# xiph/rav1e

Measured on AMD Instinct MI355X. Metric: RDO-candidate Mpixels/s (dist+fwd_tx+mc) at 4K speed-6, higher is better.
Workload: dtype u8

## Files before the change

rav1e_amd/csrc/cand_common.hpp:

```cpp
#pragma once
#include <type_traits>

#include "common.hpp"
#include "dist_common.hpp"
#include "mc_common.hpp"

namespace r1cand {

#include "mc_taps_packed.inc"

template <int CTRL>
__device__ __forceinline__ int32_t dpp(int32_t x) {
  return __builtin_amdgcn_update_dpp(0, x, CTRL, 0xf, 0xf, true);
}
template <int CTRL>
__device__ __forceinline__ int32_t bfly_lanes(int32_t x, int32_t sm) {
  return __mul24(x, sm | 1) + dpp<CTRL>(x);
}
struct LaneSigns { int32_t s1, s2; };
template <int TS>
__device__ __forceinline__ LaneSigns lane_signs(int lane) {
  LaneSigns s;
  if constexpr (TS == 8) {
    s.s1 = -(int32_t)((lane ^ (lane >> 2)) & 1);
    s.s2 = -(int32_t)(((lane >> 1) ^ (lane >> 2)) & 1);
  } else {
    s.s1 = -(int32_t)(lane & 1);
    s.s2 = 0;
  }
  return s;
}
template <int TS>
__device__ __forceinline__ uint32_t habs_lanes(int32_t x, LaneSigns sg) {
  x = bfly_lanes<0xB1>(x, sg.s1);
  if constexpr (TS == 8) x = bfly_lanes<0x4E>(x, sg.s2);
  const int32_t ax = iabs32(x);
  const int32_t ap = TS == 8 ? dpp<0x141>(ax) : dpp<0x4E>(ax);
  return (uint32_t)(ax > ap ? ax : ap);
}

__device__ __forceinline__ uint32_t sad_u32(uint32_t a, uint32_t b, uint32_t acc) {
  uint32_t r;
  asm("v_sad_u32 %0, %1, %2, %3" : "=v"(r) : "v"(a), "v"(b), "v"(acc));
  return r;
}

typedef short v2s_t __attribute__((ext_vector_type(2)));
typedef unsigned short v2us_t __attribute__((ext_vector_type(2)));
__device__ __forceinline__ uint32_t pk_add(uint32_t a, uint32_t b) {
  return __builtin_bit_cast(uint32_t, (v2s_t)(__builtin_bit_cast(v2s_t, a) + __builtin_bit_cast(v2s_t, b)));
}
__device__ __forceinline__ uint32_t pk_sub(uint32_t a, uint32_t b) {
  return __builtin_bit_cast(uint32_t, (v2s_t)(__builtin_bit_cast(v2s_t, a) - __builtin_bit_cast(v2s_t, b)));
}
__device__ __forceinline__ uint32_t pk_mad(uint32_t x, uint32_t s, uint32_t p) {
  uint32_t r;
  asm("v_pk_mad_i16 %0, %1, %2, %3" : "=v"(r) : "v"(x), "v"(s), "v"(p));
  return r;
}
__device__ __forceinline__ uint32_t pk_max(uint32_t a, uint32_t b) {
  uint32_t r;
  asm("v_pk_max_i16 %0, %1, %2" : "=v"(r) : "v"(a), "v"(b));
  return r;
}
__device__ __forceinline__ uint32_t pk_min(uint32_t a, uint32_t b) {
  uint32_t r;
  asm("v_pk_min_i16 %0, %1, %2" : "=v"(r) : "v"(a), "v"(b));
  return r;
}
__device__ __forceinline__ uint32_t pk_pair(int32_t lo, int32_t hi) {
  return __builtin_amdgcn_perm((uint32_t)hi, (uint32_t)lo, 0x05040100u);
}
__device__ __forceinline__ void pk_bfly8_s2(const uint32_t (&a)[8], uint32_t (&d)[8]) {
  uint32_t b[8];
#pragma unroll
  for (int k = 0; k < 4; k++) {
    b[2 * k] = pk_add(a[2 * k], a[2 * k + 1]);
    b[2 * k + 1] = pk_sub(a[2 * k], a[2 * k + 1]);
  }
  d[0] = pk_add(b[0], b[2]); d[2] = pk_sub(b[0], b[2]);
  d[1] = pk_add(b[1], b[3]); d[3] = pk_sub(b[1], b[3]);
  d[4] = pk_add(b[4], b[6]); d[6] = pk_sub(b[4], b[6]);
  d[5] = pk_add(b[5], b[7]); d[7] = pk_sub(b[5], b[7]);
}
__device__ __forceinline__ uint32_t habs_lanes_pk(uint32_t x, uint32_t m1, uint32_t m2, uint32_t acc) {
  x = pk_mad(x, m1, (uint32_t)dpp<0xB1>((int32_t)x));
  x = pk_mad(x, m2, (uint32_t)dpp<0x4E>((int32_t)x));
  const uint32_t ax = pk_max(x, pk_sub(0u, x));
  const uint32_t mx = pk_max(ax, (uint32_t)dpp<0x141>((int32_t)ax));
  return __builtin_amdgcn_udot2(__builtin_bit_cast(v2us_t, mx), __builtin_bit_cast(v2us_t, 0x00010001u),
                                acc, false);
}

__device__ __forceinline__ uint32_t ashr_pair(int32_t lo, int32_t hi, int sh) {
  return __builtin_amdgcn_perm((uint32_t)(hi >> sh), (uint32_t)(lo >> sh), 0x05040100u);
}

__device__ __forceinline__ int32_t dot2_seed0(uint32_t a, uint32_t b) {
  int32_t r;
  asm("v_dot2_i32_i16 %0, %1, %2, 0" : "=v"(r) : "v"(a), "v"(b));
  return r;
}
__device__ __forceinline__ int32_t dot2_seed64(uint32_t a, uint32_t b) {
  int32_t r;
  asm("v_dot2_i32_i16 %0, %1, %2, 64" : "=v"(r) : "v"(a), "v"(b));
  return r;
}
__device__ __forceinline__ int32_t dot2_seed(uint32_t a, uint32_t b, int32_t c_uniform) {
  int32_t r;
  asm("v_dot2_i32_i16 %0, %1, %2, %3" : "=v"(r) : "v"(a), "v"(b), "s"(c_uniform));
  return r;
}
__device__ __forceinline__ int32_t dot4_seed(uint32_t a, uint32_t b, int32_t c_uniform) {
  int32_t r;
  asm("v_dot4_i32_i8 %0, %1, %2, %3" : "=v"(r) : "v"(a), "v"(b), "s"(c_uniform));
  return r;
}

template <int BPP> struct Taps;
template <> struct Taps<1> { uint32_t fx0, fx1, ty[4]; };
template <> struct Taps<2> { uint32_t tx[4], ty[4]; };
template <int BPP, int W, int H>
__device__ __forceinline__ Taps<BPP> load_taps(int cf, int rf, int mx, int my) {
  const int fxi = r1mc::filter_index(mx, W), fyi = r1mc::filter_index(my, H);
  Taps<BPP> t;
  if constexpr (BPP == 1) {
    t.fx0 = kTapI8[fxi][cf][0];
    t.fx1 = kTapI8[fxi][cf][1];
  }
#pragma unroll
  for (int j = 0; j < 4; j++) {
    if constexpr (BPP == 2) t.tx[j] = kTapI16[fxi][cf][j];
    t.ty[j] = kTapI16[fyi][rf][j];
  }
  return t;
}
__device__ __forceinline__ bool taps_six(const Taps<1> &t) {
  return __all(((t.ty[0] & 0xffffu) | (t.ty[3] >> 16)) == 0);
}
__device__ __forceinline__ bool taps_six(const Taps<2> &t) {
  return __all(((t.ty[0] & 0xffffu) | (t.ty[3] >> 16) | (t.tx[0] & 0xffffu) | (t.tx[3] >> 16)) == 0);
}

#define R1_ODD_ROW_TAPS(ty, tz)                                                                   \
  do {                                                                                            \
    tz[0] = ty[0] << 16;                                                                          \
    _Pragma("unroll") for (int j = 1; j < 4; j++) tz[j] = __builtin_amdgcn_alignbit(ty[j], ty[j - 1], 16); \
    tz[4] = ty[3] >> 16;                                                                          \
  } while (0)

typedef int v4i_t __attribute__((ext_vector_type(4)));
template <int W, int H, int WS, bool PREP, bool PACK4 = false, int MXNC = 0, bool MX4 = false>
__device__ __forceinline__ void mc8_column_t(const uint8_t *win, int c, const Taps<1> &tp, int32_t *pred, bool six,
                                             int lane = 0, const uint8_t *zero = nullptr) {
  const uint32_t fx0 = tp.fx0, fx1 = tp.fx1;
  uint32_t ty[4], tz[5];
#pragma unroll
  for (int j = 0; j < 4; j++) ty[j] = tp.ty[j];
// ... 141 lines not shown
    auto hpair = [&](int r) -> uint32_t {
      if (r + 1 < H + 7) return ashr_pair(hacc(r), hacc(r + 1), hsh);
      return (uint32_t)(hacc(r) >> hsh);
    };
    uint32_t pk[5];
    pk[0] = SIX ? (uint32_t)(hacc(1) >> hsh) << 16 : hpair(0);
#pragma unroll
    for (int j = 1; j < 4; j++) pk[j] = hpair(2 * j);
#pragma unroll
    for (int j = 0; j < H / 2; j++) {
      if (!SIX || j + 1 < H / 2) pk[4] = hpair(2 * j + 8);
      int32_t a0 = PREP ? dot2_seed64(pk[0], ty[0]) : dot2_seed0(pk[0], ty[0]);
#pragma unroll
      for (int k = 1; k < 4; k++)
        a0 = __builtin_amdgcn_sdot2(__builtin_bit_cast(v2s_t, pk[k]), __builtin_bit_cast(v2s_t, ty[k]), a0, false);
      int32_t a1;
      if constexpr (SIX) {
        a1 = PREP ? dot2_seed64(pk[1], tz[1]) : dot2_seed0(pk[1], tz[1]);
#pragma unroll
        for (int k = 2; k < 4; k++)
          a1 = __builtin_amdgcn_sdot2(__builtin_bit_cast(v2s_t, pk[k]), __builtin_bit_cast(v2s_t, tz[k]), a1, false);
      } else {
        a1 = PREP ? dot2_seed64(pk[0], tz[0]) : dot2_seed0(pk[0], tz[0]);
#pragma unroll
        for (int k = 1; k < 5; k++)
          a1 = __builtin_amdgcn_sdot2(__builtin_bit_cast(v2s_t, pk[k]), __builtin_bit_cast(v2s_t, tz[k]), a1, false);
      }
      if constexpr (PREP) {
        pred[2 * j] = (a0 >> 7) - 8192;
        pred[2 * j + 1] = (a1 >> 7) - 8192;
      } else {
        a0 >>= vsh;
        a1 >>= vsh;
        pred[2 * j] = a0 < 0 ? 0 : (a0 > maxv ? maxv : a0);
        pred[2 * j + 1] = a1 < 0 ? 0 : (a1 > maxv ? maxv : a1);
      }
#pragma unroll
      for (int k = 0; k < 4; k++) pk[k] = pk[k + 1];
    }
  };
  if (six) body(std::true_type{});
  else body(std::false_type{});
}

template <int BPP, int W, int H, int WS, bool PREP, bool PACK4 = false, int MXNC = 0, bool MX4 = false>
__device__ __forceinline__ void mc_column_fast(const uint8_t *win, int c, const Taps<BPP> &tp, int bit_depth,
                                               int32_t *pred, bool six, int lane = 0, const uint8_t *zero = nullptr) {
  static_assert(!PACK4 || BPP == 1, "8 * mid of 16-bit pixels does not fit i16");
  static_assert((MXNC == 0 && !MX4) || BPP == 1, "there is no i16 matrix type");
  if constexpr (BPP == 1) mc8_column_t<W, H, WS, PREP, PACK4, MXNC, MX4>(win, c, tp, pred, six, lane, zero);
  else mc16_column_t<W, H, WS, PREP>(win, c, tp, bit_depth, pred, six);
}

__device__ __forceinline__ void satd_rows16_s2(const int32_t *v, uint32_t (&d)[8]) {
  uint32_t a[8];
#pragma unroll
  for (int k = 0; k < 8; k++) a[k] = pk_pair(v[k], v[8 + k]);
  pk_bfly8_s2(a, d);
}
template <int W, int H>
__device__ __forceinline__ void satd_tile_store(const int32_t *v, uint32_t *tcol) {
#pragma unroll
  for (int g = 0; g < H / 16; g++) {
    uint32_t d[8];
    satd_rows16_s2(v + g * 16, d);
#pragma unroll
    for (int k = 0; k < 4; k++) {
      tcol[(g * 8 + 2 * k) * W] = pk_add(d[k], d[k + 4]);
      tcol[(g * 8 + 2 * k + 1) * W] = pk_sub(d[k], d[k + 4]);
    }
  }
}
template <int NI, int P>
__device__ __forceinline__ uint32_t satd_tile_rows(const uint32_t *tile, int c) {
  uint32_t acc = 0;
#pragma unroll
  for (int m = 0; m < NI; m++) {
    const uint4 *p = (const uint4 *)(tile + (c + m * P) * 8);
    const uint4 lo = p[0], hi = p[1];
    const uint32_t x[8] = {lo.x, lo.y, lo.z, lo.w, hi.x, hi.y, hi.z, hi.w};
    uint32_t z[8];
    pk_bfly8_s2(x, z);
#pragma unroll
    for (int k = 0; k < 4; k++) {
      const uint32_t mx = pk_max(pk_max(z[k], z[k + 4]), pk_sub(0u, pk_min(z[k], z[k + 4])));
      acc = __builtin_amdgcn_udot2(__builtin_bit_cast(v2us_t, mx), __builtin_bit_cast(v2us_t, 0x00020002u), acc, false);
    }
  }
  return acc;
}

template <int TS, int H, int BD>
__device__ __forceinline__ uint32_t satd_column(const int32_t *v, int lane) {
  const LaneSigns sg = lane_signs<TS>(lane);
  uint32_t acc = 0;
  if constexpr (TS == 8 && BD <= 10) {
    const uint32_t m1 = (uint32_t)sg.s1 | 0x00010001u, m2 = (uint32_t)sg.s2 | 0x00010001u;
    if constexpr (H == 8) {
      uint32_t a[4];
#pragma unroll
      for (int k = 0; k < 4; k++) a[k] = pk_pair(v[k] + v[k + 4], v[k] - v[k + 4]);
      const uint32_t a0 = pk_add(a[0], a[1]), a1 = pk_sub(a[0], a[1]);
      const uint32_t a2 = pk_add(a[2], a[3]), a3 = pk_sub(a[2], a[3]);
      acc = habs_lanes_pk(pk_add(a0, a2), m1, m2, acc);
      acc = habs_lanes_pk(pk_add(a1, a3), m1, m2, acc);
      acc = habs_lanes_pk(pk_sub(a0, a2), m1, m2, acc);
      acc = habs_lanes_pk(pk_sub(a1, a3), m1, m2, acc);
    } else {
#pragma unroll
      for (int g = 0; g < H / 16; g++) {
        uint32_t d[8];
        satd_rows16_s2(v + g * 16, d);
#pragma unroll
        for (int k = 0; k < 4; k++) {
          acc = habs_lanes_pk(pk_add(d[k], d[k + 4]), m1, m2, acc);
          acc = habs_lanes_pk(pk_sub(d[k], d[k + 4]), m1, m2, acc);
        }
      }
    }
    return acc;
  }
#pragma unroll
  for (int g = 0; g < H / TS; g++) {
    int32_t a[TS];
#pragma unroll
    for (int k = 0; k < TS; k++) a[k] = v[g * TS + k];
    if constexpr (TS == 4) {
      const int32_t a0 = a[0] + a[1], a1 = a[0] - a[1];
      const int32_t a2 = a[2] + a[3], a3 = a[2] - a[3];
      a[0] = a0 + a2; a[1] = a1 + a3; a[2] = a0 - a2; a[3] = a1 - a3;
    } else {
      int32_t b[8], d[8];
#pragma unroll
      for (int k = 0; k < 4; k++) {
        b[2 * k] = a[2 * k] + a[2 * k + 1];
        b[2 * k + 1] = a[2 * k] - a[2 * k + 1];
      }
      d[0] = b[0] + b[2]; d[2] = b[0] - b[2];
      d[1] = b[1] + b[3]; d[3] = b[1] - b[3];
      d[4] = b[4] + b[6]; d[6] = b[4] - b[6];
      d[5] = b[5] + b[7]; d[7] = b[5] - b[7];
#pragma unroll
      for (int k = 0; k < 4; k++) {
        a[k] = d[k] + d[k + 4];
        a[k + 4] = d[k] - d[k + 4];
      }
    }
#pragma unroll
    for (int k = 0; k < TS; k++) acc += habs_lanes<TS>(a[k], sg);
  }
  return acc;
}

}
```

rav1e_amd/csrc/rdo_cand_kernel.hpp:

```cpp
#pragma once
#include <cstdlib>
#include <type_traits>

#include "cand_common.hpp"
#include "dist_common.hpp"
#include "intra_pred_common.hpp"
#include "itx_common.hpp"
#include "mc_common.hpp"
#include "quant_common.hpp"
#include "rdo_cand_args.hpp"
#include "tx_common.hpp"

#ifdef R1_PHASE_PROF
static __device__ unsigned long long g_phase[4096][8];
#define R1_PROF(i)                                                          \
  do {                                                                      \
    const unsigned long long t_ = __builtin_readcyclecounter();             \
    if (QM == 0 && threadIdx.x == 0 && (blockIdx.x & 63) == 0 && (blockIdx.x >> 6) < 4096) \
      g_phase[blockIdx.x >> 6][i] = t_ - tprev_;                            \
    tprev_ = t_;                                                            \
  } while (0)
#define R1_PROF_INIT unsigned long long tprev_ = __builtin_readcyclecounter()
#else
#define R1_PROF(i) do {} while (0)
#define R1_PROF_INIT do {} while (0)
#endif

namespace {
using r1tx::T;
using r1cand::sad_u32;

template <int BD, int WL, int HL, typename CT, int QM, bool MT = false, int PS = 0>
__global__ __launch_bounds__(64, rdo_waves_hint(BD, WL, HL, QM, MT)) void k_rdo_cand(
    R1Plane org, R1Plane ref, const R1RdoCand *__restrict__ cands, int n,
    uint32_t *__restrict__ sad_out, uint32_t *__restrict__ satd_out,
    CT *__restrict__ coeffs, void *__restrict__ pred_out, RdoQuantArgs qa,
    typename std::conditional<PS == 1, RdoIntraArgs, RdoNoIntraArgs>::type ia) {
  using PL = RdoCandPlan<BD, WL, HL, QM, MT, PS>;
  constexpr int BPP = PL::BPP, W = PL::W, H = PL::H, P = PL::P, NC = PL::NC, TS = PL::TS, WS = PL::WS, FL = PL::FL, HU = PL::HU;
  constexpr bool INTRA = PL::INTRA, SPLIT_T = PL::SPLIT_T, SRC_LDS = PL::SRC_LDS, SRC_LATE = PL::SRC_LATE,
                 SRC_KEEP = PL::SRC_KEEP, SATD_T = PL::SATD_T, COLSHARE = PL::COLSHARE;
  typedef typename PL::TB TB;
  constexpr int LSTRIDE = PL::LSTRIDE, ISTRIDE = PL::ISTRIDE, QT_STRIDE = PL::QT_STRIDE, SRC_ROW = PL::SRC_ROW,
                SRC_CSTRIDE = PL::SRC_CSTRIDE, SATD_STRIDE = PL::SATD_STRIDE, LDS_WORK = PL::LDS_WORK,
                SRC_OFF = PL::SRC_OFF, TKEEP_OFF = PL::TKEEP_OFF, LDS_BYTES = PL::LDS_BYTES;
  static_assert(!INTRA || LDS_BYTES <= RdoCandPlan<BD, WL, HL, QM, MT, 0>::LDS_BYTES,
                "an intra instantiation's LDS must not exceed its inter twin's");
  constexpr int SH0 = r1tx::fwd_shift_ct(WL, HL, BD, 0), SH1 = r1tx::fwd_shift_ct(WL, HL, BD, 1),
                SH2 = r1tx::fwd_shift_ct(WL, HL, BD, 2);
  constexpr bool COL_FOLD = PL::COL_FOLD;
  static_assert(!COL_FOLD || SH0 > 0, "the column family starts from a pending shift[0]");
  constexpr int SH1C = COL_FOLD ? 0 : SH1;
  constexpr bool HALVE2 = PL::HALVE2, MC_PACK4 = PL::MC_PACK4;
  constexpr bool MUL_HW = PL::MUL_HW;
  constexpr int CB = rdo_mul_col_bound(BD, SH0, COL_FOLD), RB = rdo_mul_row_bound(BD, WL, HL);
  constexpr int MX_NC = PL::MX_NC;
  static_assert(MX_NC == 0 || (BPP == 1 && QM == 0 && !INTRA && P == W && NC * W == 64),
                "a coefficient kernel of 8-bit pixels, lane = (candidate, column) with no idle lane");
  constexpr bool MC_MATRIX4 = PL::MC_MATRIX4;
  static_assert(!MC_MATRIX4 || (BPP == 1 && QM == 0 && !INTRA && P == W && NC * W == 64),
                "a coefficient kernel of 8-bit pixels, lane = (candidate, column) with no idle lane");
  __shared__ __attribute__((aligned(16))) uint8_t smem[LDS_BYTES];
  T *buf = (T *)smem;
  TB *tbuf = (TB *)smem;
  TB *tkeep = COLSHARE ? (TB *)(smem + TKEEP_OFF) : tbuf;

  R1_PROF_INIT;
  const unsigned wg = xcd_contiguous_wg();
  if ((long long)wg * NC >= (long long)n) return;
  const int lane = threadIdx.x;
  const int cl = lane / P, c = lane % P;
  const int cand_i = (int)wg * NC + cl;
  const long long cand = cand_i;
  constexpr bool UNMASK = !(BD == 8 && WL == 6 && HL == 6);
  const bool live_st = cand_i < n;
  static_assert(!MC_MATRIX4 || UNMASK, "the 4x4x4 MFMAs take operands from all 64 lanes: dead slots repeat a candidate");
  const bool live = UNMASK || live_st;
  const int cl_ld = live_st ? cl : n - 1 - (int)wg * NC;
  const long long cand_ld = live_st ? cand : (long long)n - 1;
  R1RdoCand cd = {};
  R1IntraCand ic = {};
  int eset = 0;
  if constexpr (INTRA) {
    if (live) {
      ic = ia.cands[cand_ld];
      eset = (int)cand_ld / ia.edge_group;
      cd.ox = ia.pos_xy[2 * eset];
      cd.oy = ia.pos_xy[2 * eset + 1];
    }
  } else {
    if (live) cd = (cands + (size_t)wg * NC)[cl_ld];
  }
#ifdef R1_PHASE_PROF
  asm volatile("s_waitcnt vmcnt(0)" ::: "memory");
  R1_PROF(5);
#endif
  constexpr bool QUANT = QM != 0;
  constexpr int PPK = QM == 2 ? (H * BPP + 3) / 4 : 1;
  uint32_t ppk[PPK];
#pragma unroll
  for (int k = 0; k < PPK; k++) ppk[k] = 0;

  T v[H];
#pragma unroll
  for (int r = 0; r < H; r++) v[r] = 0;
  const bool col_live = live && c < W;
  const uint8_t *src_l = smem + SRC_OFF + cl * SRC_CSTRIDE + c * BPP;
  constexpr int CHS = SRC_ROW >= 16 ? 16 : SRC_ROW;
  constexpr int CPR = SRC_ROW / CHS;
  constexpr int RPP = P / CPR;
  constexpr int SPASS = SRC_LDS ? (H + RPP - 1) / RPP : 1;
  const int srow = c / CPR, sch = c - srow * CPR;
  U32x4 q[SPASS];
  if constexpr (SRC_LDS) {
    const uint8_t *po = (const uint8_t *)org.data +
                        (((uint32_t)(org.yorigin + cd.oy) * (uint32_t)org.stride + (uint32_t)(org.xorigin + cd.ox)) * BPP +
                         (uint32_t)(sch * CHS));
    const uint32_t so = (uint32_t)org.stride * BPP;
#pragma unroll
    for (int u = 0; u < SPASS; u++) {
      const int rr = srow + u * RPP;
      q[u] = U32x4{0, 0, 0, 0};
      if (live && rr < H) {
        if constexpr (CHS == 16) q[u] = ld_u32x4(po + rr * so);
        else if constexpr (CHS == 8) { const U32x2 t = ld_u32x2(po + rr * so); q[u].a = t.a; q[u].b = t.b; }
        else q[u].a = ld_u32(po + rr * so);
      }
    }
  } else if (col_live) {
    const uint8_t *po = px_addr<BPP>(org, cd.ox + c, cd.oy);
    const size_t so = (size_t)org.stride * BPP;
#pragma unroll
    for (int r = 0; r < H; r++) v[r] = ld_px<BPP>(po + r * so);
  }
  uint8_t *win = smem + cl * (H + 7) * WS;
  const bool from_ref = !INTRA && live && !qa.pred_in;
  r1mc::WindowStage<BPP, BPP == 1 ? 0x80808080u : 0u, W, H, P> wst;
  if (from_ref) wst.load(ref, cd.rx, cd.ry, c);
  r1cand::Taps<BPP> tp = {};
  if (from_ref) tp = r1cand::load_taps<BPP, W, H>(cd.col_frac, cd.row_frac, cd.mode_x, cd.mode_y);
  const bool six = r1cand::taps_six(tp);
  if constexpr (PL::MX_ZERO_BYTES != 0) {
#pragma unroll
    for (int k = 0; k < (PL::MX_ZERO_BYTES / 16 + 63) / 64; k++)
      if (lane + 64 * k < PL::MX_ZERO_BYTES / 16)
        *(uint4 *)(smem + PL::MX_ZERO_OFF + 16 * (lane + 64 * k)) = make_uint4(0u, 0u, 0u, 0u);
  }
  auto stage_source = [&]() {
    if (live) {
      uint8_t *sd = smem + SRC_OFF + cl * SRC_CSTRIDE + sch * CHS;
#pragma unroll
      for (int u = 0; u < SPASS; u++) {
        const int rr = srow + u * RPP;
        if (rr < H) {
          if constexpr (CHS == 16) *(uint4 *)(sd + rr * SRC_ROW) = make_uint4(q[u].a, q[u].b, q[u].c, q[u].d);
          else if constexpr (CHS == 8) *(uint2 *)(sd + rr * SRC_ROW) = make_uint2(q[u].a, q[u].b);
          else *(uint32_t *)(sd + rr * SRC_ROW) = q[u].a;
        }
      }
    }
  };
  if constexpr (SRC_LDS && !SRC_LATE && !INTRA) stage_source();
  if (from_ref) wst.store(win, WS);
  uint16_t *eraw = (uint16_t *)smem + cl * (5 * FL);
  int left_len = 0, above_len = 0;
  if constexpr (INTRA) {
    if (live) {
      left_len = ia.lens[2 * eset];
      above_len = ia.lens[2 * eset + 1];
      const uint8_t *e = (const uint8_t *)ia.edges + ((size_t)eset * ia.edge_stride + (2 * r1ip::MAXTX - (W + H))) * BPP;
      for (int k = c; k < FL; k += P) eraw[k] = (uint16_t)ld_px<BPP>(e + k * BPP);
    }
  }
#ifdef R1_PHASE_PROF
  asm volatile("s_waitcnt vmcnt(0)" ::: "memory");
  R1_PROF(6);
#endif
  __syncthreads();
  R1_PROF(0);

  uint32_t sad_acc = 0;
  if constexpr (INTRA) {
    const bool directional = live && r1ip::is_directional(ic.mode, ic.angle);
    const bool enable = directional && ic.ief != 0;
    const uint16_t *tl = eraw + (W + H);
    uint16_t *work = eraw + FL;
    int up_a = 0, up_l = 0;
    r1ip::edge_filter_upsample<const R1IntraCand &>(tl, 0, work, W, H, P, c, ic, enable, left_len, above_len,
                                                     (1 << BD) - 1, up_a, up_l);
    int32_t pred[H];
    if (col_live) {
      if (ic.mode == r1ip::UV_CFL_PRED && !ia.ac) ic.angle = 0;
      const int16_t *acb = ic.mode == r1ip::UV_CFL_PRED && ia.ac ? ia.ac + (size_t)cand_ld * (W * H) : nullptr;
      r1ip::predict_column<const R1IntraCand &>(W, H, c, ic, directional, enable, up_a, up_l, tl, 0, work, left_len, BD,
                                                 acb, [&](int i, int32_t pv) { pred[i] = pv; });
      if (pred_out && live_st) {
        if constexpr (BPP == 1) {
          uint8_t *pp = (uint8_t *)pred_out + (size_t)cand * W * H + c;
#pragma unroll
          for (int r = 0; r < H; r++) pp[(size_t)r * W] = (uint8_t)pred[r];
        } else {
          uint16_t *pp = (uint16_t *)pred_out + (size_t)cand * W * H + c;
#pragma unroll
          for (int r = 0; r < H; r++) pp[(size_t)r * W] = (uint16_t)pred[r];
        }
      }
      if constexpr (QM == 2) {
#pragma unroll
        for (int r = 0; r < H; r++) {
          if constexpr (BPP == 1) ppk[r >> 2] |= (uint32_t)pred[r] << (8 * (r & 3));
          else ppk[r >> 1] |= (uint32_t)pred[r] << (16 * (r & 1));
        }
      }
    }
    if constexpr (SRC_LDS) {
      __syncthreads();
      stage_source();
      __syncthreads();
    }
    if (col_live) {
      if constexpr (SRC_LDS) {
#pragma unroll
        for (int r = 0; r < H; r++) {
          const uint32_t sp = BPP == 1 ? (uint32_t)src_l[r * SRC_ROW] : (uint32_t) * (const uint16_t *)(src_l + r * SRC_ROW);
          sad_acc = sad_u32(sp, (uint32_t)pred[r], sad_acc);
          v[r] = (T)sp - pred[r];
        }
      } else {
#pragma unroll
        for (int r = 0; r < H; r++) v[r] -= pred[r];
      }
    }
  } else
  if constexpr (BPP == 1) {
    if (col_live) {
      int32_t pred[H];
      if (qa.pred_in) {
        const uint8_t *pi = (const uint8_t *)qa.pred_in + (size_t)cand_ld * W * H + c;
#pragma unroll
        for (int r = 0; r < H; r++) pred[r] = pi[(size_t)r * W];
      } else {
        if constexpr (MX_NC != 0)
          r1cand::mc_column_fast<BPP, W, H, WS, false, MC_PACK4, MX_NC>(smem, c, tp, BD, pred, six, lane,
                                                                         smem + PL::MX_ZERO_OFF);
        else if constexpr (MC_MATRIX4)
          r1cand::mc_column_fast<BPP, W, H, WS, false, MC_PACK4, 0, true>(win, c, tp, BD, pred, six);
        else
        r1cand::mc_column_fast<BPP, W, H, WS, false, MC_PACK4>(win, c, tp, BD, pred, six);
      }
      if (pred_out && live_st) {
        uint8_t *pp = (uint8_t *)pred_out + (size_t)cand * W * H + c;
#pragma unroll
        for (int r = 0; r < H; r++) pp[(size_t)r * W] = (uint8_t)pred[r];
      }
      if constexpr (QM == 2) {
#pragma unroll
        for (int r = 0; r < H; r++) ppk[r >> 2] |= (uint32_t)pred[r] << (8 * (r & 3));
      }
      if constexpr (SRC_LDS) {
#pragma unroll
        for (int r = 0; r < H; r++) {
          const uint32_t sp = src_l[r * SRC_ROW];
          sad_acc = sad_u32(sp, (uint32_t)pred[r], sad_acc);
          v[r] = (T)sp - pred[r];
        }
      } else {
#pragma unroll
        for (int r = 0; r < H; r++) v[r] -= pred[r];
      }
    }
  } else {
    int32_t pred[H];
    if (col_live) {
      if (qa.pred_in) {
        const uint16_t *pi = (const uint16_t *)qa.pred_in + (size_t)cand_ld * W * H + c;
#pragma unroll
        for (int r = 0; r < H; r++) pred[r] = pi[(size_t)r * W];
      } else {
        r1cand::mc_column_fast<BPP, W, H, WS, false>(win, c, tp, BD, pred, six);
      }
      if (pred_out && live_st) {
        uint16_t *pp = (uint16_t *)pred_out + (size_t)cand * W * H + c;
#pragma unroll
        for (int r = 0; r < H; r++) pp[(size_t)r * W] = (uint16_t)pred[r];
      }
      if constexpr (QM == 2) {
#pragma unroll
        for (int r = 0; r < H; r++) ppk[r >> 1] |= (uint32_t)pred[r] << (16 * (r & 1));
      }
    }
    if constexpr (SRC_LATE) {
      __syncthreads();
      stage_source();
      __syncthreads();
    }
    if (col_live) {
      if constexpr (SRC_LDS) {
#pragma unroll
        for (int r = 0; r < H; r++) {
          const uint32_t sp = *(const uint16_t *)(src_l + r * SRC_ROW);
          sad_acc = sad_u32(sp, (uint32_t)pred[r], sad_acc);
          v[r] = (T)sp - pred[r];
        }
      } else {
#pragma unroll
        for (int r = 0; r < H; r++) v[r] -= pred[r];
      }
    }
  }
  R1_PROF(1);
  if (sad_out) {
    uint32_t sad = sad_acc;
    if constexpr (!SRC_LDS) {
#pragma unroll
      for (int r = 0; r < H; r++) sad += (uint32_t)iabs32(v[r]);
    }
    const uint32_t s = group_sum<P>(sad);
    if (live_st && c == 0) (sad_out + (size_t)wg * NC)[cl] = s;
  }
  if (satd_out) {
    uint32_t part;
    if constexpr (SATD_T) {
      uint32_t *tile = (uint32_t *)smem + cl * SATD_STRIDE;
      __syncthreads();
      if (c < W) r1cand::satd_tile_store<W, H>(v, tile + c);
      __syncthreads();
      part = r1cand::satd_tile_rows<(W < H ? W : H) / 16, P>(tile, c);
    } else {
      part = r1cand::satd_column<TS, H, BD>(v, lane);
    }
    const uint32_t s = group_sum<P>(part);
    constexpr int LN = TS == 4 ? 2 : 3;
    if (live_st && c == 0) (satd_out + (size_t)wg * NC)[cl] = (s + ((1u << LN) >> 1)) >> LN;
  }
  R1_PROF(2);
  if (!QUANT && !coeffs) return;

  constexpr bool MT_RECOMP = MT && SRC_KEEP;
  T vkeep[MT && !MT_RECOMP ? H : 1];
  if constexpr (MT && !MT_RECOMP) {
#pragma unroll
    for (int r = 0; r < H; r++) vkeep[r] = v[r];
  }
  constexpr bool TAIL_DEFER = MT && QM == 2 && W == 8 && H == 8;
  const bool tail_defer = TAIL_DEFER && qa.dist_kind == R1_DIST_CDEF && qa.nt <= 8;
  r1dist::CdefMoments tail_keep;
  uint32_t rem = MT ? qa.tx_mask : 1u;
  bool fresh = true;
  do {
  int t0 = 0;
  uint32_t gmask = 1u;
  if constexpr (MT) {
    t0 = (int)__builtin_ctz(rem);
    gmask = 1u << t0;
    if constexpr (COLSHARE) {
      auto colkey = [](int t) { return r1tx::vtx_1d(t) | ((int)r1tx::ud_flip(t) << 4) | ((int)r1tx::lr_flip(t) << 5); };
      const int k0 = colkey(t0);
      for (uint32_t m = rem & (rem - 1); m != 0; m &= m - 1) {
        const int t = (int)__builtin_ctz(m);
        if (colkey(t) == k0) gmask |= 1u << t;
      }
    }
    rem &= ~gmask;
    if (!fresh) {
      if constexpr (MT_RECOMP) {
        if (col_live) {
#pragma unroll
          for (int r = 0; r < H; r++) {
            const T sp = BPP == 1 ? (T)src_l[r * SRC_ROW] : (T) * (const uint16_t *)(src_l + r * SRC_ROW);
            const T pr = BPP == 1 ? (T)((ppk[r >> 2] >> (8 * (r & 3))) & 0xFF)
                                  : (T)((ppk[r >> 1] >> (16 * (r & 1))) & 0xFFFF);
            v[r] = sp - pr;
          }
        }
      } else {
#pragma unroll
        for (int r = 0; r < H; r++) v[r] = vkeep[r];
      }
    }
    fresh = false;
  }
  __syncthreads();
  const int tx_col = MT ? t0 : (QM != 0 && qa.tx_mask != 0 ? (int)__builtin_ctz(qa.tx_mask) : (int)cd.tx_type);
  constexpr bool TX_VOTE = rdo_tx_vote(WL, HL, QM, MT, PS);
  static_assert(!TX_VOTE || UNMASK, "the vote reads every lane's descriptor");
  int tx_s = 0;
  bool tx_uni = false, col_uni = false, row_uni = false;
  if constexpr (TX_VOTE) {
    tx_s = __builtin_amdgcn_readfirstlane(tx_col);
    tx_uni = __all(tx_col == tx_s);
    col_uni = tx_uni && r1tx::vtx_1d(tx_s) != 3;
    row_uni = tx_uni && r1tx::htx_1d(tx_s) != 3;
  }
  bool any_ud;
  if (TX_VOTE && tx_uni) any_ud = r1tx::ud_flip(tx_s);
  else any_ud = __any(live && r1tx::ud_flip(tx_col));
  if (col_live) {
    if (any_ud) {
      const bool ud = r1tx::ud_flip(tx_col);
#pragma unroll
      for (int r = 0; r < H / 2; r++) {
        const T t0 = v[r], t1 = v[H - 1 - r];
        v[r] = ud ? t1 : t0;
        v[H - 1 - r] = ud ? t0 : t1;
      }
    }
    if constexpr (COL_FOLD) {
      if constexpr (MUL_HW) {
        if (TX_VOTE && col_uni) r1tx::fwd_col_m24w_kernel<H, SH0, SH1, CB>(v, r1tx::vtx_1d(tx_s));
        else r1tx::fwd_col_m24w<H, SH0, SH1, CB>(v, r1tx::vtx_1d(tx_col));
      } else {
        if (TX_VOTE && col_uni) r1tx::fwd_col_m24_kernel<H, SH0, SH1, HALVE2>(v, r1tx::vtx_1d(tx_s));
        else r1tx::fwd_col_m24<H, SH0, SH1, HALVE2>(v, r1tx::vtx_1d(tx_col));
      }
    } else {
#pragma unroll
      for (int r = 0; r < H; r++) v[r] = r1tx::shift_fwd_ct<SH0>(v[r]);
      if constexpr (MUL_HW) {
        if (TX_VOTE && col_uni) r1tx::fwd_1d_m24w_kernel<H, CB>(v, r1tx::vtx_1d(tx_s));
        else r1tx::fwd_1d_m24w<H, CB>(v, r1tx::vtx_1d(tx_col));
      } else {
        if (TX_VOTE && col_uni) r1tx::fwd_1d_m24_kernel<H, HALVE2>(v, r1tx::vtx_1d(tx_s));
        else r1tx::fwd_1d_m24<H, HALVE2>(v, r1tx::vtx_1d(tx_col));
      }
    }
    if constexpr (!SPLIT_T) {
      const int cc = cl * W + (r1tx::lr_flip(tx_col) ? W - 1 - c : c);
#pragma unroll
      for (int r = 0; r < HU; r++)
        tkeep[r * LSTRIDE + cc] = (TB)r1tx::shift_fwd_ct<SH1C>(v[r]);
    }
  }
  if constexpr (!SPLIT_T) __syncthreads();
  R1_PROF(3);
  do {
  const int tx_type = MT ? (int)__builtin_ctz(gmask) : tx_col;
  const int slot = MT ? (int)__builtin_popcount(qa.tx_mask & ((1u << tx_type) - 1u)) : 0;
  const long long oslot = MT ? cand * (long long)qa.nt + slot
                             : (QM != 0 && qa.nt != 0 ? cand * (long long)qa.nt + qa.slot : cand);
  const int cl2 = cl, r = c;
  const bool live2 = live;
  const bool row_live = live2 && r < HU;
  const int tt = tx_type;
  constexpr int OS = H < 32 ? H : 32, WC = W < 32 ? W : 32;
  T u[W];
  if constexpr (SPLIT_T) {
    const int cc = r1tx::lr_flip(tx_type) ? W - 1 - c : c;
#pragma unroll
    for (int half = 0; half < HU / 32; half++) {
      if (col_live) {
#pragma unroll
        for (int rr = 0; rr < 32; rr++)
          tbuf[rr * LSTRIDE + cc] = (TB)r1tx::shift_fwd_ct<SH1C>(v[half * 32 + rr]);
      }
      __syncthreads();
      if (row_live && (r >> 5) == half) {
#pragma unroll
        for (int k = 0; k < W; k++) u[k] = tbuf[(r & 31) * LSTRIDE + k];
      }
      __syncthreads();
    }
  }
  if (row_live) {
    if constexpr (!SPLIT_T) {
#pragma unroll
      for (int k = 0; k < W; k++) u[k] = tkeep[r * LSTRIDE + cl2 * W + k];
    }
    if constexpr (MUL_HW) {
      if (TX_VOTE && row_uni) r1tx::fwd_1d_m24w_kernel<W, RB>(u, r1tx::htx_1d(tx_s));
      else r1tx::fwd_1d_m24w<W, RB>(u, r1tx::htx_1d(tt));
    } else {
      if (TX_VOTE && row_uni) r1tx::fwd_1d_m24_kernel<W, HALVE2>(u, r1tx::htx_1d(tx_s));
      else r1tx::fwd_1d_m24<W, HALVE2>(u, r1tx::htx_1d(tt));
    }
#pragma unroll
    for (int k = 0; k < W; k++) {
      u[k] = r1tx::shift_fwd_ct<SH2>(u[k]);
      if constexpr (QUANT) u[k] = (T)(CT)u[k];
    }
  }
  if constexpr (MT) {
  } else
  if constexpr (P > 16) {
    if (coeffs && row_live && live_st) {
// ... 311 lines not shown
```

rav1e_amd/csrc/rdo_cand_plan.hpp:

```cpp
#pragma once
#include <cstdint>
#include <type_traits>

#include "mc_window.hpp"

constexpr int rdo_waves_hint(int bd, int wl, int hl, int qm, bool mt = false) {
  if (mt) {
    if (wl <= 3 && hl <= 3) return qm == 2 ? (bd == 8 ? 7 : 6) : 1;
    return qm == 2 ? 4 : 1;
  }
  if (wl == 5 && hl == 5 && qm == 0 && bd != 8) return 6;
  if (wl == 3 && hl == 3 && qm == 2) return 8;
  if (wl == 4 && hl == 4 && qm == 2) return bd == 8 ? 6 : 5;
  if (wl == 5 && hl == 5 && qm == 2) return 4;
  if (wl == 5 && hl == 5 && qm == 1) return 5;
  if (wl == 6 && hl == 6 && qm == 2) return bd == 8 ? 4 : 3;
  return 1;
}

constexpr bool rdo_tx_size_exists(int wl, int hl) {
  return wl >= 2 && wl <= 6 && hl >= 2 && hl <= 6 && wl - hl <= 2 && hl - wl <= 2;
}
constexpr bool rdo_type_fanout(int wl, int hl) { return wl <= 4 && hl <= 4; }
constexpr bool r1_intra_two_launch(int wl, int hl, int bd, int qm) {
  return wl == hl && ((wl == 4 && (qm == 1 || bd != 8)) || (wl == 6 && qm == 1 && bd != 8) ||
                      (wl == 5 && qm == 2 && bd != 8));
}
enum RdoIntraRoute { RDO_INTRA_FANOUT, RDO_INTRA_PER_TYPE, RDO_INTRA_TWO_LAUNCH };
constexpr RdoIntraRoute rdo_intra_route(int wl, int hl, int bd, int qm) {
  return r1_intra_two_launch(wl, hl, bd, qm) ? RDO_INTRA_TWO_LAUNCH
                                             : (rdo_type_fanout(wl, hl) ? RDO_INTRA_FANOUT : RDO_INTRA_PER_TYPE);
}
constexpr bool rdo_cand_instantiated(int bd, int wl, int hl, int qm, bool mt, int ps) {
  if (!(bd == 8 || bd == 10 || bd == 12) || !rdo_tx_size_exists(wl, hl) || qm < 0 || qm > 2 || ps < 0 || ps > 1)
    return false;
  if (ps == 1)
    return qm != 0 && rdo_intra_route(wl, hl, bd, qm) == (mt ? RDO_INTRA_FANOUT : RDO_INTRA_PER_TYPE);
  return !mt || (qm != 0 && rdo_type_fanout(wl, hl));
}

constexpr bool rdo_tx_vote(int wl, int hl, int qm, bool mt, int ps) {
  return qm == 0 && !mt && ps == 0 && wl <= 4 && hl <= 4;
}

constexpr bool rdo_col_fold(int bd, int wl, int hl, int qm, bool mt, int ps) {
  if (mt || ps != 0 || wl != hl) return false;
  if (bd == 8) return qm == 0 ? (wl >= 3 && wl <= 5) : (qm == 1 && (wl == 3 || wl == 4));
  return bd == 10 && qm == 0 && (wl == 4 || wl == 5);
}

constexpr bool rdo_plain_square(int wl, int hl, int qm, bool mt, int ps) {
  return qm == 0 && !mt && ps == 0 && wl == hl && wl >= 3 && wl <= 6;
}
constexpr bool rdo_halve2(int bd, int wl, int hl, int qm, bool mt, int ps) {
  if (!rdo_plain_square(wl, hl, qm, mt, ps)) return false;
  return bd == 8 || (bd == 10 && (wl == 4 || wl == 6));
}
constexpr bool rdo_mc_pack4(int bd, int wl, int hl, int qm, bool mt, int ps) {
  return bd == 8 && rdo_plain_square(wl, hl, qm, mt, ps) && wl <= 5;
}
constexpr bool rdo_mul_hiword_built(int bd, int wl, int hl, int qm, bool mt, int ps) {
  return bd == 8 && rdo_plain_square(wl, hl, qm, mt, ps);
}
constexpr bool rdo_mul_hiword(int bd, int wl, int hl, int qm, bool mt, int ps) {
  return rdo_mul_hiword_built(bd, wl, hl, qm, mt, ps);
}
constexpr int rdo_mul_col_bound(int bd, int sh0, bool col_fold) { return ((1 << bd) - 1) << (col_fold ? 0 : sh0); }
constexpr int rdo_mul_row_bound(int bd, int wl, int hl) {
  return bd == 8 && wl == hl ? (wl == 3 ? 5774 : wl == 4 ? 8164 : wl == 5 ? 5776 : wl == 6 ? 16334 : 0) : 0;
}
constexpr bool rdo_mc_matrix(int bd, int wl, int hl, int qm, bool mt, int ps) {
  return bd == 8 && rdo_plain_square(wl, hl, qm, mt, ps) && wl >= 5;
}
constexpr bool rdo_mc_matrix4_layout(int bd, int wl, int hl, int qm, bool mt, int ps) {
  return bd == 8 && rdo_plain_square(wl, hl, qm, mt, ps) && (wl == 4 || wl == 3);
}
constexpr bool rdo_mc_matrix4(int bd, int wl, int hl, int qm, bool mt, int ps) {
  return rdo_mc_matrix4_layout(bd, wl, hl, qm, mt, ps) && (wl == 4 || wl == 3);
}

template <int BD, int WL, int HL, int QM, bool MT, int PS>
struct RdoCandPlan {
  static constexpr int BPP = BD == 8 ? 1 : 2;
  static constexpr bool INTRA = PS == 1;
  static constexpr int W = 1 << WL, H = 1 << HL;
  static constexpr int P = W > H ? W : H, NC = 64 / P;
  static constexpr int TS = (W < H ? W : H) == 4 ? 4 : 8;
  static constexpr bool COL_FOLD = rdo_col_fold(BD, WL, HL, QM, MT, PS);
  static constexpr bool HALVE2 = rdo_halve2(BD, WL, HL, QM, MT, PS);
  static constexpr bool MC_PACK4 = rdo_mc_pack4(BD, WL, HL, QM, MT, PS);
  static constexpr bool MUL_HW = rdo_mul_hiword(BD, WL, HL, QM, MT, PS);
  static_assert(!MUL_HW || (HALVE2 && rdo_mul_row_bound(BD, WL, HL) > 0), "m24w keeps m24h's halving; a stated row bound");
  static constexpr int WS = r1mc::window_stride(W, BPP);
  static constexpr int WIN_BYTES = INTRA ? 0 : NC * (H + 7) * WS;
  static constexpr int FL = 2 * (W + H) + 1;
  static constexpr int EDGE_BYTES = INTRA ? ((NC * 5 * FL * 2 + 15) & ~15) : 0;
  static constexpr bool TB16 = (BD == 10 && WL == 5 && HL == 5) || (MT && W <= 16 && H <= 16);
  typedef typename std::conditional<TB16, int16_t, int32_t>::type TB;
  static constexpr int LSTRIDE = NC * W + (TB16 ? 2 : 1);
  static constexpr int ISTRIDE = NC * W + 1;
  static constexpr bool SPLIT_T = W == 64 && H == 64;
  static constexpr int TXB_ROWS = SPLIT_T ? 32 : H;
  static constexpr int TXB_BYTES = TXB_ROWS * LSTRIDE * (int)sizeof(TB);
  static constexpr int IRB_BYTES = QM == 2 ? (H < 32 ? H : 32) * ISTRIDE * 4 : 0;
  static constexpr int QT_PAD = NC > 2 ? P : 0;
  static constexpr int QT_STRIDE = (W < 32 ? W : 32) * (H < 32 ? H : 32) + QT_PAD;
  static constexpr int QT_BYTES = QM != 0 ? NC * QT_STRIDE * 4 : 0;
  static constexpr int HU = (QM == 2 && H > 32) ? 32 : H;
  static constexpr int REC_BYTES = QM == 2 ? NC * W * H * BPP : 0;
  static constexpr bool SRC_LDS = BPP == 1 || P <= 32;
  static constexpr bool SRC_LATE0 = SRC_LDS && BD != 8 && (P == 32 || (P == 16 && QM == 0));
  static constexpr int SRC_ROW = W * BPP;
  static constexpr int WIN_PAD = (WIN_BYTES + 15) & ~15;
  static constexpr int SRC_CSTRIDE = H * SRC_ROW + (NC > 1 ? (SRC_ROW > 16 ? SRC_ROW : 16) : 0);
  static constexpr int SRC_BYTES = SRC_LDS ? NC * SRC_CSTRIDE : 0;
  static constexpr bool SRC_KEEP = QM == 2 && H <= 16 && SRC_LDS && !SRC_LATE0;
  static constexpr bool SRC_LATE = INTRA ? SRC_LDS && !SRC_KEEP : SRC_LATE0;
  static constexpr int WS_BYTES =
      SRC_KEEP ? WIN_PAD : (SRC_LATE ? (WIN_PAD > SRC_BYTES ? WIN_PAD : SRC_BYTES) : WIN_PAD + SRC_BYTES);
  static constexpr int LDS_A0 = WS_BYTES > TXB_BYTES ? WS_BYTES : TXB_BYTES;
  static constexpr int LDS_A = LDS_A0 > IRB_BYTES ? LDS_A0 : IRB_BYTES;
  static constexpr int SATD_STRIDE = W * H / 2 + (NC > 1 ? P : 0);
  static constexpr int SATD_BYTES = NC * SATD_STRIDE * 4;
  static constexpr bool SATD_T = TS == 8 && BD <= 10 && (W < H ? W : H) >= 16 && SATD_BYTES <= LDS_A &&
                                 !(QM == 2 && WL == 6 && HL == 6);
  static_assert(SATD_STRIDE % 4 == 0, "16-byte reads stay aligned");
  static constexpr int LDS_B = QT_BYTES > REC_BYTES ? QT_BYTES : REC_BYTES;
  static constexpr int LDS_WORK = ((LDS_A > LDS_B ? LDS_A : LDS_B) + 15) & ~15;
  static constexpr int SRC_OFF = SRC_KEEP ? LDS_WORK : (SRC_LATE ? 0 : WIN_PAD);
  static constexpr bool COLSHARE = MT && !SPLIT_T;
  static constexpr int TKEEP_OFF = (LDS_WORK + (SRC_KEEP ? SRC_BYTES : 0) + 15) & ~15;
  static constexpr int LDS_CHAIN =
      COLSHARE ? TKEEP_OFF + H * LSTRIDE * (int)sizeof(TB) : LDS_WORK + (SRC_KEEP ? SRC_BYTES : 0);
  static constexpr int LDS_BYTES = LDS_CHAIN > EDGE_BYTES ? LDS_CHAIN : EDGE_BYTES;
  static constexpr bool MC_MATRIX = rdo_mc_matrix(BD, WL, HL, QM, MT, PS);
  static constexpr int MX_NC = MC_MATRIX ? NC : 0;
  static constexpr int MX_ZERO_BYTES = MC_MATRIX && NC > 1 ? r1mc::mx_zero_bytes(H, WS) : 0;
  static constexpr int MX_ZERO_OFF = (WIN_PAD + SRC_BYTES + 15) & ~15;
  static_assert(!MC_MATRIX || (NC <= 2 && WS % 8 == 0 && !SRC_LATE && !SRC_KEEP && SRC_OFF == WIN_PAD),
                "the matrix pass reads aligned 8-byte fragments of one or two windows; the shadow follows the source");
  static_assert(!MC_MATRIX || r1mc::mx_a_end(NC > 2 ? 2 : NC, H, WS) <= LDS_BYTES,
                "the furthest byte an A fragment reads lies inside the allocation");
  static_assert(!MC_MATRIX || MX_ZERO_OFF + MX_ZERO_BYTES <= LDS_BYTES, "the zeroed shadow lies inside the allocation");
  static constexpr bool MC_MATRIX4 = rdo_mc_matrix4(BD, WL, HL, QM, MT, PS);
  static constexpr int MX4_A_END = rdo_mc_matrix4_layout(BD, WL, HL, QM, MT, PS) ? r1mc::mx4_a_end(NC, W, H, WS) : 0;
  static_assert(!MC_MATRIX4 || !MC_MATRIX, "one matrix form per instantiation");
  static_assert(MX4_A_END == 0 || (NC * W == 64 && W % 4 == 0 && WS % 4 == 0 && WS >= W + 8 && !SRC_LATE),
                "lane = (candidate, column) with no idle lane; a block is four columns of one candidate; its three "
                "dwords stay inside the row");
  static_assert(MX4_A_END <= LDS_BYTES, "the furthest byte an A fragment reads lies inside the allocation");
};
```

Measured before the change: 738,700.

## Compute 64x64 8-bit SATD with int8 MFMA Hadamard transforms

```diff
diff --git a/rav1e_amd/csrc/cand_common.hpp b/rav1e_amd/csrc/cand_common.hpp
--- a/rav1e_amd/csrc/cand_common.hpp
+++ b/rav1e_amd/csrc/cand_common.hpp
@@ -4,6 +4,7 @@
 #include "common.hpp"
 #include "dist_common.hpp"
 #include "mc_common.hpp"
+#include "satd_matrix.hpp"
 
 namespace r1cand {
 
@@ -451,4 +452,38 @@
   return acc;
 }
 
-}
+__device__ __forceinline__ uint32_t sad_bias(uint32_t d, uint32_t bias_uniform, uint32_t acc) {
+  return __builtin_amdgcn_sad_u16(d, bias_uniform, acc);
+}
+static __constant__ r1sx::HTable kSatdH = r1sx::HTable();
+template <int W, int NC, int CSTRIDE, int SRC_OFF>
+__device__ __forceinline__ uint32_t satd_matrix(const uint8_t *blocks, int lane) {
+  const uint4 hf = *(const uint4 *)kSatdH.w[lane];
+  long a[2][2];
+  a[0][0] = (long)(((uint64_t)hf.y << 32) | hf.x);
+  a[1][0] = (long)(((uint64_t)hf.w << 32) | hf.z);
+  a[0][1] = (long)r1sx::h_negate((uint64_t)a[0][0]);
+  a[1][1] = (long)r1sx::h_negate((uint64_t)a[1][0]);
+  const uint8_t *bl = blocks + r1sx::b_lane(lane, W, NC, CSTRIDE);
+  const v4i_t cbias = {r1sx::BIAS, r1sx::BIAS, r1sx::BIAS, r1sx::BIAS};
+  uint32_t acc = 0;
+#pragma unroll
+  for (int t = 0; t < r1sx::groups(NC); t++) {
+    long b[r1sx::CHUNKS];
+#pragma unroll
+    for (int k = 0; k < r1sx::CHUNKS; k++)
+      b[k] = *(const long *)(bl + (k < 2 ? SRC_OFF : 0) + r1sx::b_step(t, k, W)) ^ (long)0x8080808080808080ull;
+#pragma unroll
+    for (int m = 0; m < r1sx::MBLOCKS; m++) {
+      v4i_t d = cbias;
+#pragma unroll
+      for (int k = 0; k < r1sx::CHUNKS; k++)
+        d = __builtin_amdgcn_mfma_i32_16x16x32_i8(a[r1sx::a_odd(m)][r1sx::a_neg(m, k)], b[k], d, 0, 0, 0);
+#pragma unroll
+      for (int i = 0; i < 4; i++) acc = sad_bias((uint32_t)d[i], (uint32_t)r1sx::BIAS, acc);
+    }
+  }
+  return acc;
+}
+
+}
diff --git a/rav1e_amd/csrc/rdo_cand_kernel.hpp b/rav1e_amd/csrc/rdo_cand_kernel.hpp
--- a/rav1e_amd/csrc/rdo_cand_kernel.hpp
+++ b/rav1e_amd/csrc/rdo_cand_kernel.hpp
@@ -75,6 +75,11 @@
   constexpr bool UNMASK = !(BD == 8 && WL == 6 && HL == 6);
   const bool live_st = cand_i < n;
   static_assert(!MC_MATRIX4 || UNMASK, "the 4x4x4 MFMAs take operands from all 64 lanes: dead slots repeat a candidate");
+  constexpr bool SATD_MX = PL::SATD_MX;
+  static_assert(!SATD_MX || (BPP == 1 && QM == 0 && !INTRA && SRC_LDS && P == W && NC * W == 64),
+                "a coefficient kernel of 8-bit pixels, lane = (candidate, column) with no idle lane");
+  static_assert(!SATD_MX || UNMASK || NC == 1,
+                "the MFMAs take operands from all 64 lanes: dead slots repeat a candidate, or one candidate per wave");
   const bool live = UNMASK || live_st;
   const int cl_ld = live_st ? cl : n - 1 - (int)wg * NC;
   const long long cand_ld = live_st ? cand : (long long)n - 1;
@@ -257,6 +262,17 @@
 #pragma unroll
         for (int r = 0; r < H; r++) ppk[r >> 2] |= (uint32_t)pred[r] << (8 * (r & 3));
       }
+      if constexpr (SATD_MX) {
+        __syncthreads();
+        uint8_t *pt = smem + cl * SRC_CSTRIDE + c;
+#pragma unroll
+        for (int r = 0; r < H; r++) {
+          const uint32_t sp = src_l[r * SRC_ROW];
+          sad_acc = sad_u32(sp, (uint32_t)pred[r], sad_acc);
+          v[r] = (T)sp - pred[r];
+          pt[r * SRC_ROW] = (uint8_t)pred[r];
+        }
+      } else
       if constexpr (SRC_LDS) {
 #pragma unroll
         for (int r = 0; r < H; r++) {
@@ -319,7 +335,16 @@
     if (live_st && c == 0) (sad_out + (size_t)wg * NC)[cl] = s;
   }
   if (satd_out) {
-    uint32_t part;
+    uint32_t part, s;
+    if constexpr (SATD_MX) {
+      __syncthreads();
+      part = r1cand::satd_matrix<W, NC, SRC_CSTRIDE, SRC_OFF>(smem, lane);
+      constexpr int CW = r1sx::cand_cols(NC);
+      part = group_sum<CW>(part);
+      part += __shfl_xor(part, 16, WAVE);
+      part += __shfl_xor(part, 32, WAVE);
+      s = __shfl(part, cl * CW, WAVE);
+    } else {
     if constexpr (SATD_T) {
       uint32_t *tile = (uint32_t *)smem + cl * SATD_STRIDE;
       __syncthreads();
@@ -329,7 +354,8 @@
     } else {
       part = r1cand::satd_column<TS, H, BD>(v, lane);
     }
-    const uint32_t s = group_sum<P>(part);
+    s = group_sum<P>(part);
+    }
     constexpr int LN = TS == 4 ? 2 : 3;
     if (live_st && c == 0) (satd_out + (size_t)wg * NC)[cl] = (s + ((1u << LN) >> 1)) >> LN;
   }
diff --git a/rav1e_amd/csrc/rdo_cand_plan.hpp b/rav1e_amd/csrc/rdo_cand_plan.hpp
--- a/rav1e_amd/csrc/rdo_cand_plan.hpp
+++ b/rav1e_amd/csrc/rdo_cand_plan.hpp
@@ -3,6 +3,7 @@
 #include <type_traits>
 
 #include "mc_window.hpp"
+#include "satd_matrix.hpp"
 
 constexpr int rdo_waves_hint(int bd, int wl, int hl, int qm, bool mt = false) {
   if (mt) {
@@ -79,6 +80,13 @@
   return rdo_mc_matrix4_layout(bd, wl, hl, qm, mt, ps) && (wl == 4 || wl == 3);
 }
 
+constexpr bool rdo_satd_matrix_layout(int bd, int wl, int hl, int qm, bool mt, int ps) {
+  return bd == 8 && rdo_plain_square(wl, hl, qm, mt, ps);
+}
+constexpr bool rdo_satd_matrix(int bd, int wl, int hl, int qm, bool mt, int ps) {
+  return rdo_satd_matrix_layout(bd, wl, hl, qm, mt, ps) && wl == 6;
+}
+
 template <int BD, int WL, int HL, int QM, bool MT, int PS>
 struct RdoCandPlan {
   static constexpr int BPP = BD == 8 ? 1 : 2;
@@ -149,4 +157,18 @@
                 "lane = (candidate, column) with no idle lane; a block is four columns of one candidate; its three "
                 "dwords stay inside the row");
   static_assert(MX4_A_END <= LDS_BYTES, "the furthest byte an A fragment reads lies inside the allocation");
+  static constexpr bool SATD_MX = rdo_satd_matrix(BD, WL, HL, QM, MT, PS);
+  static constexpr bool SATD_MX_LAYOUT = rdo_satd_matrix_layout(BD, WL, HL, QM, MT, PS);
+  static constexpr int SX_PRED_BYTES = SATD_MX_LAYOUT ? NC * SRC_CSTRIDE : 0;
+  static constexpr int SX_B_END = SATD_MX_LAYOUT ? r1sx::b_end(W, NC, SRC_CSTRIDE) : 0;
+  static_assert(!SATD_MX || SATD_MX_LAYOUT, "what ships has a stated layout");
+  static_assert(!SATD_MX_LAYOUT || (BPP == 1 && W == H && NC * W == 64 && SRC_LDS && !SRC_LATE && !SRC_KEEP &&
+                                    SRC_OFF == WIN_PAD && SRC_ROW == W),
+                "lane = (candidate, column) with no idle lane; the source block behind the window, rows of W bytes");
+  static_assert(!SATD_MX_LAYOUT || (SRC_OFF % 8 == 0 && SRC_CSTRIDE % 8 == 0 && W % 8 == 0), "8-byte reads stay aligned");
+  static_assert(SX_PRED_BYTES <= SRC_OFF && SX_B_END <= SX_PRED_BYTES && SX_B_END <= SRC_BYTES,
+                "the prediction tile ends before the source block; every fragment lies inside its region");
+  static_assert(!SATD_MX_LAYOUT || (r1sx::pred_write(63, H - 1, W, SRC_CSTRIDE) < SX_PRED_BYTES &&
+                                    SRC_OFF + SRC_BYTES <= LDS_BYTES),
+                "the furthest byte written and the furthest byte read lie inside the allocation");
 };
diff --git a/rav1e_amd/csrc/satd_matrix.hpp b/rav1e_amd/csrc/satd_matrix.hpp
--- /dev/null
+++ b/rav1e_amd/csrc/satd_matrix.hpp
@@ -0,0 +1,57 @@
+#pragma once
+#include <cstdint>
+
+namespace r1sx {
+
+constexpr int BIAS = 16384;
+constexpr int CHUNKS = 4, MBLOCKS = 4;
+
+constexpr int groups(int nc) { return nc == 1 ? 4 : (nc == 2 ? 2 : 1); }
+constexpr int cand_cols(int nc) { return nc == 8 ? 1 : 16 / nc; }
+constexpr int col_cand(int j, int nc) { return nc == 8 ? (j & 7) : j / cand_cols(nc); }
+constexpr bool col_live(int j, int nc) { return nc < 8 || j < 8; }
+constexpr int col_tile(int t, int j, int nc) { return nc == 8 ? 0 : cand_cols(nc) * t + j % cand_cols(nc); }
+
+constexpr int pred_write(int l, int r, int w, int cstride) { return (l / w) * cstride + r * w + l % w; }
+constexpr int b_offset(int l, int t, int k, int w, int nc, int cstride) {
+  const int j = l & 15, g = l >> 4, tile = col_tile(t, j, nc), tpr = w / 8;
+  return col_cand(j, nc) * cstride + (8 * (tile / tpr) + 4 * (k & 1) + g) * w + 8 * (tile % tpr);
+}
+constexpr int b_lane(int l, int w, int nc, int cstride) { return b_offset(l, 0, 0, w, nc, cstride); }
+constexpr int b_step(int t, int k, int w) { return (16 * t + 4 * (k & 1)) * w; }
+constexpr int b_end(int w, int nc, int cstride) {
+  int e = 0;
+  for (int l = 0; l < 64; l++) {
+    const int o = b_offset(l, groups(nc) - 1, 1, w, nc, cstride) + 8;
+    e = o > e ? o : e;
+  }
+  return e;
+}
+
+constexpr uint64_t h_frag(int l, int odd) {
+  const int j = l & 15, g = l >> 4, v = j & 7;
+  uint64_t f = 0;
+  for (int x = 0; x < 8; x++) {
+    const int vx = v & x;
+    const int neg = ((vx ^ (vx >> 1) ^ (vx >> 2)) ^ ((j >> 3) & g) ^ (odd & (g >> 1))) & 1;
+    f |= (uint64_t)(neg ? 0xffu : 0x01u) << (8 * x);
+  }
+  return f;
+}
+constexpr uint64_t h_negate(uint64_t f) { return f ^ 0xfefefefefefefefeull; }
+constexpr int a_odd(int m) { return m & 1; }
+constexpr bool a_neg(int m, int k) { return ((((m >> 1) & k) ^ (k >> 1)) & 1) != 0; }
+
+struct HTable {
+  uint32_t w[64][4];
+  constexpr HTable() : w{} {
+    for (int l = 0; l < 64; l++)
+      for (int odd = 0; odd < 2; odd++) {
+        const uint64_t f = h_frag(l, odd);
+        w[l][2 * odd] = (uint32_t)f;
+        w[l][2 * odd + 1] = (uint32_t)(f >> 32);
+      }
+  }
+};
+
+}
```

Result: no change. 737,000, median of 3 (-0.2%).
